# emsig/emg3d

Hardware: AMD Instinct MI355X
Metric: Mcells*smoother-iters/s (fp64) per multigrid cycle (higher is better)
Workload: dtype c128 (complex fp64)

## Files before the change

### emg3d_amd/csrc/kernels.hip

```cpp
#include <hip/hip_runtime.h>

#include <algorithm>
#include <climits>
#include <cstdio>
#include <cstdlib>
#include <cstring>
#include <string>
#include <type_traits>

#include "../../include/emg3d_amd.h"
#include "launch.h"

using emg::cplx;

namespace {

thread_local std::string g_err;

int fail(int code, const char *what)
{
    g_err = what;
    return code;
}

// ... 952 lines not shown
        else if (rq == 2) A.E(1)[A.idx(1, mk + 1, i1, i2)] = xq;
        else if (rq == 3) A.E(2)[A.idx(2, mk + 1, i1, i2 - 1)] = xq;
        else if (rq == 4) A.E(2)[A.idx(2, mk + 1, i1, i2)] = xq;
        else A.E(0)[A.idx(0, mk + 1, i1, i2)] = xq;
    }
    WSTAMP(5);
    __syncthreads();
    WSTAMP(6);
    {
        const int nst = (half ? nbb : nbt) - 1;
        if (chain_wave && nst > 0) {
            const int kb0 = half ? mk + 2 : mk - 1, dk = half ? 1 : -1;
            T *const rw = GH + (size_t)cl * rows * LW_ROW;
            const T v0 = rw[kb0 * LW_ROW + (lane & 3)];
            wide_chain<T, true>(rw, nbase, nrow, (unsigned)cl * 16, kb0 + dk, kb0, dk, nst, lane & 15, v0);
        }
    }
    WSTAMP(7);
    __syncthreads();
    WSTAMP(8);
    if (has && !isq) {
        const T *const hr = GH + ((size_t)ll * rows + k) * LW_ROW;
        T h[4], c[5], x[5];
#pragma unroll
        for (int q = 0; q < 4; ++q) h[q] = hr[q];
#pragma unroll
        for (int q = 0; q < 5; ++q) c[q] = r[q];
        emg::wide_x<T, 15>(Tk, c, h, x);
        emg::wide_block_scatter<T, DIR>(A, k, mir, i1, i2, x);
    }
    WSTAMP(9);
}

template <class T, int DIR>
__device__ __forceinline__ void stream_produce(const emg::Axes<T, DIR> &A, int colour, int cntp, int cntq, int n0p,
                                               int line0, int nl, int lpw, T *buf, int R, int chunk, int pt, int np,
                                               double *lfo = nullptr)
{
    const int n0 = A.n0();
    const int items = 2 * R * lpw;
    for (int it = pt; it < items; it += np) {
        int ll, row, half;
        if (DIR == 0) { row = it % R; ll = (it / R) % lpw; half = it / (R * lpw); }
        else { ll = it % lpw; row = (it / lpw) % R; half = it / (R * lpw); }
        const int i = chunk * R + row;
        const int k = half ? n0p - 1 - i : i;
        const int k0 = k, kt = half ? k - 1 : k;
        const int lid = line0 + min(ll, nl - 1);
        int i1, i2, l2;
        emg::line_of_thread<DIR>(colour, cntp, cntq, lid % cntp, lid / cntp, i1, i2, l2);
        T rhs[5];
        emg::line_rhs_t<T, DIR>(A, min(max(kt, 0), n0 - 1), i1, i2, rhs);
        rhs[0] = emg::line_rhs_e0<T, DIR>(A, min(max(k0, 0), n0 - 1), i1, i2);
        const double keep0 = (k0 >= 0 && k0 < n0) ? 1.0 : 0.0;
        const double keept = (kt >= 0 && kt < n0) ? 1.0 : 0.0;
        T *o = buf + ((size_t)(half * R + row) * lpw + ll) * 5;
        o[0] = keep0 * rhs[0];
#pragma unroll
        for (int r = 1; r < 5; ++r) o[r] = keept * rhs[r];
        if (lfo) {
            double c[8];
            emg::line_coupling<T, DIR>(A, k, i1, i2, half != 0, c);
            double *lo = lfo + ((size_t)(half * R + row) * lpw + ll) * 8;
#pragma unroll
            for (int r = 0; r < 8; ++r) lo[r] = c[r];
        }
    }
}

constexpr int stream_producers(int B, bool compact) { return (B >= 2 || compact) ? 384 : 256; }
constexpr int stream_depth(int dir, int B, bool compact) { return B >= 2 ? 2 : (compact && dir == 0) ? 8 : emg::LINE_PAD; }
constexpr bool stream_lf_ring(int B) { return B == 1; }

template <class T, int HALF, int RD, int B, class FT = T, class WT = T>
__device__ __forceinline__ void quad_forward_stream(int n0, int n0p, int nlines, int qline, int qend, int line0, int j,
                                                      const FT *fac, const double *lfac, WT *vec, size_t vstride,
                                                      size_t dummy_off, const T *ringbase, int lpw, int R, int nchunks,
                                                      const double *lfring)
{
    const HalfWalk<HALF> W(n0, n0p);
    const bool active = qline < qend;
    const int line = min(qline, qend - 1);
    const int ll = line - line0;
    const VecRef<WT> V = VecRef<WT>::global(vec, nlines);
    WT *const dummy = vec + dummy_off;
    WT *const dslot = dummy + ((threadIdx.x & 63) >> 2) * 5;
    constexpr bool LFR = stream_lf_ring(B);
    QuadRow<T, FT> ring[RD];
    using LAddr = LaneAddr<T, HALF, FT, WT>;
    const LAddr LA(fac, lfac, nlines, line, j, V);
    auto fetch = [&](QuadRow<T, FT> &q, int i) { q.template load<LAddr, false, !LFR>(LA, W.fwd(W.clampi(i))); };
#pragma unroll
    for (int d = 0; d < RD; ++d) fetch(ring[d], d);
    __syncthreads();
    T wsel[B], w4p[B];
#pragma unroll
    for (int b = 0; b < B; ++b) wsel[b] = w4p[b] = emg::zero<T>();
    const double nz = j != 0 ? 1.0 : 0.0, is0 = 1.0 - nz;
    const size_t srcelems = (size_t)2 * R * lpw * 5;
    const size_t bufelems = (size_t)B * srcelems;
    for (int c = 0; c < nchunks; ++c) {
        const T *const items = ringbase + (size_t)(c & 1) * bufelems + ((size_t)(HALF * R) * lpw + ll) * 5;
        const int iend = min((c + 1) * R, W.steps);
        for (int i0 = c * R; i0 < iend; i0 += RD) {
#pragma unroll
            for (int d = 0; d < RD; ++d) {
                const int k = W.fwd(i0 + d);
                QuadRow<T, FT> &q = ring[d];
                const T *const it = items + (size_t)(i0 + d - c * R) * lpw * 5;
                if constexpr (LFR)
                    q.take_b(lfring + (size_t)(c & 1) * ((size_t)2 * R * lpw * 8) +
                             ((size_t)(HALF * R + (i0 + d - c * R)) * lpw + ll) * 8, j);
                WT *const o4 = active ? LA.pv4(k) : dslot + 4;
                WT *const oj = active ? LA.pvj(k) : dslot + j;
#pragma unroll
                for (int b = 0; b < B; ++b) {
                    const T v = it[b * srcelems + j], v4 = it[b * srcelems + 4];
                    T wn, w4;
                    quad_forward_step(q, v, v4, nz, is0, wsel[b], w4p[b], wn, w4);
                    oj[b * vstride] = emg::narrow<WT>(wn);
                    o4[b * vstride] = emg::narrow<WT>(w4);
                }
                fetch(ring[d], i0 + d + RD);
            }
        }
        lds_barrier();
    }
}

template <class T, int DIR, class WT = T>
__device__ __forceinline__ void stream_produce_w(const WT *vec, int nlines, int n0, int n0p, int line0, int nl, int lpw,
                                                 T *buf, int R, int chunk, int pt, int np,
                                                 const emg::Axes<T, DIR> *A = nullptr, int colour = 0, int cntp = 0,
                                                 int cntq = 0, double *lfo = nullptr)
{
    const int mk = emg::line_mid(n0);
    const int items = 2 * R * lpw;
    for (int it = pt; it < items; it += np) {
        const int ll = it % lpw, row = (it / lpw) % R, half = it / (R * lpw);
        const int steps = half ? n0p - 2 - mk : mk;
        const int ic = max(min(chunk * R + row, steps - 1), 0);
        const int k = min(max(half ? mk + 2 + ic : mk - 1 - ic, half), n0p - 1);
        const int lid = line0 + min(ll, nl - 1);
        const WT *const r0 = vec + ((size_t)k * nlines + lid) * 5;
        const WT *const rt = vec + ((size_t)(half ? k - 1 : k) * nlines + lid) * 5;
        const WT a0 = r0[0], a1 = rt[1], a2 = rt[2], a3 = rt[3], a4 = rt[4];
        T *o = buf + ((size_t)(half * R + row) * lpw + ll) * 5;
        o[0] = emg::widen(a0); o[1] = emg::widen(a1); o[2] = emg::widen(a2); o[3] = emg::widen(a3); o[4] = emg::widen(a4);
        if (lfo) {
            int i1, i2, l2;
            emg::line_of_thread<DIR>(colour, cntp, cntq, lid % cntp, lid / cntp, i1, i2, l2);
            double c[8];
            emg::line_coupling<T, DIR>(*A, k, i1, i2, half != 0, c);
            double *lo = lfo + ((size_t)(half * R + row) * lpw + ll) * 8;
#pragma unroll
            for (int r = 0; r < 8; ++r) lo[r] = c[r];
        }
    }
}

template <class T, int DIR, int HALF, int RD, int B, class FT = T, class WT = T>
__device__ __forceinline__ void quad_backward_stream(const emg::Level<T> &L, int colour, int cntp, int cntq, int n0p, int qline,
                                                int qend, int line0, int j, const FT *fac, const double *lfac, WT *vec,
                                                size_t vstride, T *fdummy, size_t boff0, const T *ringbase, int lpw, int R,
                                                int nchunks, const double *lfring)
{
    const emg::Axes<T, DIR> A(L, boff0);
    const int n0 = A.n0();
    const HalfWalk<HALF> W(n0, n0p);
    const int mk = W.mk;
    const int nlines = cntp * cntq;
    const bool active = qline < qend;
    const int line = min(qline, qend - 1);
    const int ll = line - line0;
    const size_t bs = L.bstride;
    int i1, i2, lid;
    emg::line_of_thread<DIR>(colour, cntp, cntq, line % cntp, line / cntp, i1, i2, lid);
    const int cj = j == 0 ? 0 : (j <= 2 ? 1 : 2), dk = (j == 0 || HALF) ? 0 : 1, dk4 = HALF ? 0 : 1;
    const int d1 = j == 1 ? 1 : 0, d2 = j == 3 ? 1 : 0;
    T *const ej = A.E(cj) + A.idx(cj, dk, i1 - d1, i2 - d2);
    const long sj = (long)A.idx(cj, dk + 1, i1 - d1, i2 - d2) - (long)A.idx(cj, dk, i1 - d1, i2 - d2);
    T *const e4 = A.E(2) + A.idx(2, dk4, i1, i2);
    const long s4 = (long)A.idx(2, dk4 + 1, i1, i2) - (long)A.idx(2, dk4, i1, i2);
    T *const dslot = fdummy + ((threadIdx.x & 63) >> 2) * 5;
    T *const dj = dslot + j, *const d4 = dslot + 4;
    const size_t fstep = active ? bs : 0;

    const VecRef<WT> V = VecRef<WT>::global(vec, nlines);
    constexpr bool LFR = stream_lf_ring(B);
    QuadRow<T, FT> ring[RD];
// ... 48 lines not shown
                QuadRow<T, FT> &q = ring[d];
                const T *const it = items + (size_t)(i0 + d - c * R) * lpw * 5;
                if constexpr (LFR)
                    q.take_b(lfring + (size_t)(c & 1) * ((size_t)2 * R * lpw * 8) +
                             ((size_t)(HALF * R + (i0 + d - c * R)) * lpw + ll) * 8, j);
                const bool real_block = HALF ? k <= n0 - 1 : true;
                T *const oj = real_block ? pej : dj;
                T *const o4 = real_block ? pe4 : d4;
                const size_t ostep = real_block ? fstep : 0;
#pragma unroll
                for (int b = 0; b < B; ++b) {
                    const T wj = it[b * srcelems + j], w4 = it[b * srcelems + 4];
                    T xn, xn4;
                    quad_backward_step(q, wj, w4, nz, upA, upD, up04, up44, x0[b], x4[b], xmine[b], xn, xn4);
                    if (PAIRED && (d & 1) == 0) {
                        hold_j[b] = xn; hold_4[b] = xn4;
                    } else if (PAIRED) {
                        hold_oj[b * hold_step] = hold_j[b];
                        oj[b * ostep] = xn;
                        hold_o4[b * hold_step] = hold_4[b];
                        o4[b * ostep] = xn4;
                    } else {
                        oj[b * ostep] = xn;
                        o4[b * ostep] = xn4;
                    }
                }
                if (PAIRED && (d & 1) == 0) { hold_oj = oj; hold_o4 = o4; hold_step = ostep; }
                upA = q.bA; upD = q.bD; up04 = q.b04; up44 = q.d4;
                pej += incj;
                pe4 += inc4;
                fetch(ring[d], i0 + d + RD);
            }
        }
        lds_barrier();
    }
}

template <class T, int DIR, int B, bool COMPACT>
__global__ __launch_bounds__(128 + stream_producers(B, COMPACT), 1) void k_line_stream(emg::Level<T> L, int colour, int cntp, int cntq, int n0p,
                                                                    int lpw, int R, const void *facv, const double *lfac,
                                                                    T *vecT, size_t vstrideT, size_t boff0)
{
    constexpr int RD = stream_depth(DIR, B, COMPACT), NPROD = stream_producers(B, COMPACT);
    constexpr bool LFR = stream_lf_ring(B);
    using FT = typename std::conditional<COMPACT, typename emg::compact_of<T>::type, T>::type;
    using WT = FT;
    const FT *const fac = reinterpret_cast<const FT *>(facv);
    WT *const vec = reinterpret_cast<WT *>(vecT);
    const size_t vstride = vstrideT * (sizeof(T) / sizeof(WT));
    const size_t dummy_off = vstrideT - emg::LINE_DUMMY;
    T *const fdummy = vecT + dummy_off;
    extern __shared__ double2 ls_smem[];
    const int nlines = cntp * cntq;
    const int line0 = blockIdx.x * lpw;
    const int nl = min(lpw, nlines - line0);
    T *const ringbase = reinterpret_cast<T *>(ls_smem);
    const size_t srcelems = (size_t)2 * R * lpw * 5, bufelems = (size_t)B * srcelems;
    double *const lfring = LFR ? reinterpret_cast<double *>(ringbase + 2 * bufelems) : nullptr;
    const size_t lfelems = (size_t)2 * R * lpw * 8;
    const int n0 = DIR == 0 ? L.nx : DIR == 1 ? L.ny : L.nz;
    const int mk = emg::line_mid(n0);
    const int smax = max(mk, n0p - 2 - mk);
    const int nchunks = (smax + R - 1) / R;
    const int wave = threadIdx.x >> 6;
    if (wave >= 2) {
        const int pt = threadIdx.x - 128;
#pragma unroll 1
        for (int b = 0; b < B; ++b) {
            const emg::Axes<T, DIR> A(L, boff0 + b * L.bstride);
            const VecRef<WT> V = VecRef<WT>::global(vec + b * vstride, nlines);
            for (int ll = pt; ll < nl; ll += NPROD) {
                const int lid = line0 + ll;
                int i1, i2, l2;
                emg::line_of_thread<DIR>(colour, cntp, cntq, lid % cntp, lid / cntp, i1, i2, l2);
                T rhs[5];
                emg::line_rhs<T, DIR>(A, mk, i1, i2, rhs);
#pragma unroll
                for (int r = 0; r < 4; ++r) *V.p(mk, lid, r) = emg::narrow<WT>(rhs[r]);
                *V.p4(mk, lid) = emg::narrow<WT>(rhs[4]);
                *V.p(mk + 1, lid, 0) = emg::narrow<WT>(emg::line_rhs_e0<T, DIR>(A, min(mk + 1, n0 - 1), i1, i2));
            }
            stream_produce<T, DIR>(A, colour, cntp, cntq, n0p, line0, nl, lpw, ringbase + b * srcelems, R, 0, pt, NPROD,
                                   (LFR && b == 0) ? lfring : nullptr);
        }
        __syncthreads();
        for (int c = 0; c < nchunks; ++c) {
            if (c + 1 < nchunks) {
#pragma unroll 1
                for (int b = 0; b < B; ++b) {
                    const emg::Axes<T, DIR> A(L, boff0 + b * L.bstride);
                    stream_produce<T, DIR>(A, colour, cntp, cntq, n0p, line0, nl, lpw,
                                           ringbase + (size_t)((c + 1) & 1) * bufelems + b * srcelems, R, c + 1, pt, NPROD,
                                           (LFR && b == 0) ? lfring + (size_t)((c + 1) & 1) * lfelems : nullptr);
                }
            }
            lds_barrier();
        }
        __syncthreads();
        const emg::Axes<T, DIR> A0(L, boff0);
#pragma unroll 1
        for (int b = 0; b < B; ++b)
            stream_produce_w<T, DIR, WT>(vec + b * vstride, nlines, n0, n0p, line0, nl, lpw, ringbase + b * srcelems, R, 0, pt, NPROD,
                                         &A0, colour, cntp, cntq, (LFR && b == 0) ? lfring : nullptr);
        __syncthreads();
        for (int c = 0; c < nchunks; ++c) {
            if (c + 1 < nchunks) {
#pragma unroll 1
                for (int b = 0; b < B; ++b)
                    stream_produce_w<T, DIR, WT>(vec + b * vstride, nlines, n0, n0p, line0, nl, lpw,
                                                 ringbase + (size_t)((c + 1) & 1) * bufelems + b * srcelems, R, c + 1, pt, NPROD,
                                                 &A0, colour, cntp, cntq,
                                                 (LFR && b == 0) ? lfring + (size_t)((c + 1) & 1) * lfelems : nullptr);
            }
            lds_barrier();
        }
        return;
    }
    const int half = wave & 1;
    const int qline = line0 + ((threadIdx.x & 63) >> 2), j = threadIdx.x & 3;
    const int qend = line0 + nl;
    if (half == 0) quad_forward_stream<T, 0, RD, B, FT, WT>(n0, n0p, nlines, qline, qend, line0, j, fac, lfac, vec, vstride, dummy_off, ringbase, lpw, R, nchunks, lfring);
    else quad_forward_stream<T, 1, RD, B, FT, WT>(n0, n0p, nlines, qline, qend, line0, j, fac, lfac, vec, vstride, dummy_off, ringbase, lpw, R, nchunks, lfring);
    __syncthreads();
    if (half == 0) quad_backward_stream<T, DIR, 0, RD, B, FT, WT>(L, colour, cntp, cntq, n0p, qline, qend, line0, j, fac, lfac, vec, vstride, fdummy, boff0, ringbase, lpw, R, nchunks, lfring);
    else quad_backward_stream<T, DIR, 1, RD, B, FT, WT>(L, colour, cntp, cntq, n0p, qline, qend, line0, j, fac, lfac, vec, vstride, fdummy, boff0, ringbase, lpw, R, nchunks, lfring);
}

#pragma clang fp contract(fast)

template <class T, bool ROLL>
__global__ __launch_bounds__(256) void k_residual(emg::Level<T> L0, T *rx, T *ry, T *rz, double *partial, int nzb, int zb)
{
    const int b = blockIdx.z / nzb;
    const emg::Level<T> L = emg::source_level(L0, b);
    if (rx) { rx += b * L0.bstride; ry += b * L0.bstride; rz += b * L0.bstride; }
    const int ix = blockIdx.x * blockDim.x + threadIdx.x;
    const int iy = blockIdx.y * blockDim.y + threadIdx.y;
    const int z0 = (blockIdx.z - b * nzb) * zb, z1 = min(z0 + zb, L.nz + 1);
    double acc = 0.0;
    if (ix <= L.nx && iy <= L.ny) {
        if constexpr (ROLL) acc = emg::residual_column<T>(L, rx, ry, rz, ix, iy, z0, z1);
        else for (int iz = z0; iz < z1; ++iz) acc += emg::residual_cell<T>(L, rx, ry, rz, ix, iy, iz);
    }
    if (partial) {
        for (int off = 32; off > 0; off >>= 1) acc += __shfl_down(acc, off, 64);
        __shared__ double wsum[4];
        const int tid = threadIdx.y * blockDim.x + threadIdx.x;
// ... 567 lines not shown
    {"line_wide_bt", &g_line_wide_bt},
    {"line_compact", &g_line_compact, -1, 1},
    {"point_compact", &g_point_compact, -1, 1},
};
constexpr int N_OPTIONS = sizeof(g_options) / sizeof(g_options[0]);
static int g_options_generation = 0;

int emg3d_option_count(void) { return N_OPTIONS; }
const char *emg3d_option_name(int i) { return (i >= 0 && i < N_OPTIONS) ? g_options[i].name : nullptr; }

int emg3d_set_option(const char *name, int value)
{
    if (!name) return fail(EMG3D_ERR_BADARG, "set_option: null name");
    for (const OptionEntry &o : g_options) {
        if (std::strcmp(name, o.name)) continue;
        if (o.value == &g_residual_zb && value < 1) value = 1;
        bool ok = value >= o.lo && value <= o.hi;
        if (o.value == &g_line_lpw) ok = value == 0 || value == 4 || value == 8 || value == 16 || value == 32;
        if (o.value == &g_line_stream_r) ok = ok && value % emg::LINE_PAD == 0;
        if (o.value == &g_line_wide_bt) ok = value == 0 || value == 192 || value == 256;
        if (!ok) {
            g_err = std::string("set_option: ") + name + " = " + std::to_string(value) + " is not an admissible value";
            return EMG3D_ERR_BADARG;
        }
        if (*o.value != value) ++g_options_generation;
        *o.value = value;
        return 0;
    }
    return fail(EMG3D_ERR_BADARG, "set_option: unknown option");
}

int emg3d_options_generation(void) { return g_options_generation; }

#ifdef EMG_WIDE_STAMPS
int emg3d_debug_wide_stamps(unsigned long long *out)
{
    return (int)hipMemcpyFromSymbol(out, HIP_SYMBOL(g_wide_stamps), sizeof(unsigned long long) * 32);
}
#endif

const char *emg3d_line_kernel_name(int lr, int nx, int ny, int nz, int is_complex, int batch)
{
    if (lr < 1 || lr > 3 || nx < 2 || ny < 2 || nz < 2) return "";
    const emg::LineClass lc = emg::line_class(lr - 1, nx, ny, nz, 3);
    if (lc.lines <= 0) return "";
    if (line_wide_used(lr - 1, nx, ny, nz)) return "k_line_wide";
    const LinePlan P = is_complex ? line_plan<cplx>(lc, batch > 1 ? batch : 1) : line_plan<double>(lc, batch > 1 ? batch : 1);
    switch (P.kind) {
    case LK_STREAM: return "k_line_stream";
    case LK_COLOUR: return "k_line_colour";
    default: return "k_line_rhs+k_line_forward+k_line_backward";
    }
}

int emg3d_get_option(const char *name)
{
    if (name)
        for (const OptionEntry &o : g_options)
            if (!std::strcmp(name, o.name)) return *o.value;
    return -1;
}

int emg3d_device_count(void)
{
    int n = 0;
    if (hipGetDeviceCount(&n) != hipSuccess) return 0;
// ... 384 lines not shown
```

### emg3d_amd/csrc/stencil.h

```cpp
#pragma once
#include "cplx.h"

namespace emg {

template <class T> struct Level {
    int nx, ny, nz;
    T *ex, *ey, *ez;
    const T *sx, *sy, *sz;
    const T *eta_x, *eta_y, *eta_z;
    const double *zeta;
    const double *ihx, *ihy, *ihz;
    int batch = 1;
    size_t bstride = 0;
    int flags = 0;
};
constexpr int LEVEL_ETA_IMAG = 1;
constexpr int LEVEL_LINE_COMPACT = 2;
constexpr int LEVEL_POINT_COMPACT = 4;
template <class T> EMG_HD Level<T> source_level(Level<T> L, int b)
{
    size_t o = (size_t)b * L.bstride;
#if defined(__HIP_DEVICE_COMPILE__)
    o = ((size_t)__builtin_amdgcn_readfirstlane((unsigned)(o >> 32)) << 32) | (size_t)__builtin_amdgcn_readfirstlane((unsigned)o);
#endif
// ... 635 lines not shown
    const double mxyLzm = k10 * (z100 + z000), mxyRzm = k11 * (z110 + z010);
    const double myxLzp = k00 * (z011 + z001), myxRzp = k01 * (z111 + z101);
    const double mxyLzp = k10 * (z101 + z001), mxyRzp = k11 * (z111 + z011);

    const T st0 = A.eta(0, i0m, i1, i2) + A.eta(0, i0m, i1, i2m) + A.eta(0, i0m, i1m, i2) +
                  A.eta(0, i0m, i1m, i2m);
    const T st2 = A.eta(1, i0, i1m, i2) + A.eta(1, i0, i1m, i2m) + A.eta(1, i0m, i1m, i2) +
                  A.eta(1, i0m, i1m, i2m);
    const T st3 = A.eta(1, i0, i1, i2) + A.eta(1, i0, i1, i2m) + A.eta(1, i0m, i1, i2) +
                  A.eta(1, i0m, i1, i2m);
    const T st4 = A.eta(2, i0, i1, i2m) + A.eta(2, i0, i1m, i2m) + A.eta(2, i0m, i1, i2m) +
                  A.eta(2, i0m, i1m, i2m);
    const T st5 = A.eta(2, i0, i1, i2) + A.eta(2, i0, i1m, i2) + A.eta(2, i0m, i1, i2) +
                  A.eta(2, i0m, i1m, i2);

    dg[0] = (mzyRxm * h11 + mzyLxm * h10 + myzRxm * h21 + myzLxm * h20) - 0.25 * st0;
    dg[1] = (mzxRym * h01 + mzxLym * h00 + mxzRym * h21 + mxzLym * h20) - 0.25 * st2;
    dg[2] = (mzxRyp * h01 + mzxLyp * h00 + mxzRyp * h21 + mxzLyp * h20) - 0.25 * st3;
    dg[3] = (myxRzm * h01 + myxLzm * h00 + mxyRzm * h11 + mxyLzm * h10) - 0.25 * st4;
    dg[4] = (myxRzp * h01 + myxLzp * h00 + mxyRzp * h11 + mxyLzp * h10) - 0.25 * st5;

    mid[1][0] = -mzyLxm * h00; mid[2][0] = mzyRxm * h00; mid[3][0] = -myzLxm * h00; mid[4][0] = myzRxm * h00;
    mid[2][1] = 0.0;
    mid[3][1] = -mxzLym * h10; mid[4][1] = mxzRym * h10;
    mid[3][2] = mxzLyp * h11; mid[4][2] = -mxzRyp * h11;
    mid[4][3] = 0.0;

    left0[0] = 0.0;
    left0[1] = mzyLxm * h00; left0[2] = -mzyRxm * h00; left0[3] = myzLxm * h00; left0[4] = -myzRxm * h00;
    leftd[0] = 0.0;
    leftd[1] = -mzxLym * h00; leftd[2] = -mzxLyp * h00; leftd[3] = -myxLzm * h00; leftd[4] = -myxLzp * h00;
}

template <class T, int DIR>
EMG_HD T line_rhs_e0(const Axes<T, DIR> &A, int k, int i1, int i2)
{
    const int i0m = k;
    const int i1m = i1 - 1, i1p = i1 + 1, i2m = i2 - 1, i2p = i2 + 1;
    const double h10 = A.ih1()[i1m], h11 = A.ih1()[i1];
    const double h20 = A.ih2()[i2m], h21 = A.ih2()[i2];
    const double k10 = 0.5 * h10, k11 = 0.5 * h11, k20 = 0.5 * h20, k21 = 0.5 * h21;
    const double z000 = A.zeta(i0m, i1m, i2m), z010 = A.zeta(i0m, i1, i2m);
    const double z001 = A.zeta(i0m, i1m, i2), z011 = A.zeta(i0m, i1, i2);
    const double mzyLxm = k10 * (z001 + z000), mzyRxm = k11 * (z011 + z010);
    const double myzLxm = k20 * (z010 + z000), myzRxm = k21 * (z011 + z001);
    T r0 = A.s(0, i0m, i1, i2);
    r0 += (mzyRxm * h11) * A.e(0, i0m, i1p, i2);
    r0 += (mzyLxm * h10) * A.e(0, i0m, i1m, i2);
    r0 += (myzRxm * h21) * A.e(0, i0m, i1, i2p);
    r0 += (myzLxm * h20) * A.e(0, i0m, i1, i2m);
    return r0;
}
template <class T, int DIR>
EMG_HD void line_rhs_t(const Axes<T, DIR> &A, int k, int i1, int i2, T (&rhs)[5])
{
    const int n0 = A.n0();
    const int i0m = k;
    const int i0 = (k + 1 < n0 - 1) ? k + 1 : n0 - 1;
    const int i1m = i1 - 1, i1p = i1 + 1, i2m = i2 - 1, i2p = i2 + 1;
    const double h00 = A.ih0()[i0m], h01 = A.ih0()[i0];
    const double h10 = A.ih1()[i1m], h11 = A.ih1()[i1];
    const double h20 = A.ih2()[i2m], h21 = A.ih2()[i2];
    const double k00 = 0.5 * h00, k01 = 0.5 * h01, k10 = 0.5 * h10, k11 = 0.5 * h11;
    const double k20 = 0.5 * h20, k21 = 0.5 * h21;

    const double z000 = A.zeta(i0m, i1m, i2m), z010 = A.zeta(i0m, i1, i2m);
    const double z001 = A.zeta(i0m, i1m, i2), z011 = A.zeta(i0m, i1, i2);
    const double z100 = A.zeta(i0, i1m, i2m), z110 = A.zeta(i0, i1, i2m);
    const double z101 = A.zeta(i0, i1m, i2), z111 = A.zeta(i0, i1, i2);
    const double mzxLym = k00 * (z001 + z000), mzxRym = k01 * (z101 + z100);
    const double mxzLym = k20 * (z100 + z000), mxzRym = k21 * (z101 + z001);
    const double mzxLyp = k00 * (z011 + z010), mzxRyp = k01 * (z111 + z110);
    const double mxzLyp = k20 * (z110 + z010), mxzRyp = k21 * (z111 + z011);
    const double myxLzm = k00 * (z010 + z000), myxRzm = k01 * (z110 + z100);
    const double mxyLzm = k10 * (z100 + z000), mxyRzm = k11 * (z110 + z010);
    const double myxLzp = k00 * (z011 + z001), myxRzp = k01 * (z111 + z101);
    const double mxyLzp = k10 * (z101 + z001), mxyRzp = k11 * (z111 + z011);

    rhs[1] = A.s(1, i0, i1m, i2);
    rhs[2] = A.s(1, i0, i1, i2);
    rhs[3] = A.s(2, i0, i1, i2m);
    rhs[4] = A.s(2, i0, i1, i2);

    rhs[1] += h10 * (mzxRym * A.e(0, i0, i1m, i2) - mzxLym * A.e(0, i0m, i1m, i2) +
                     mxzRym * A.e(2, i0, i1m, i2) - mxzLym * A.e(2, i0, i1m, i2m));
    rhs[1] += (mxzRym * h21) * A.e(1, i0, i1m, i2p);
    rhs[1] += (mxzLym * h20) * A.e(1, i0, i1m, i2m);

    rhs[2] += h11 * (mzxLyp * A.e(0, i0m, i1p, i2) - mzxRyp * A.e(0, i0, i1p, i2) +
                     mxzLyp * A.e(2, i0, i1p, i2m) - mxzRyp * A.e(2, i0, i1p, i2));
    rhs[2] += (mxzRyp * h21) * A.e(1, i0, i1, i2p);
    rhs[2] += (mxzLyp * h20) * A.e(1, i0, i1, i2m);

    rhs[3] += h20 * (myxRzm * A.e(0, i0, i1, i2m) - myxLzm * A.e(0, i0m, i1, i2m) +
                     mxyRzm * A.e(1, i0, i1, i2m) - mxyLzm * A.e(1, i0, i1m, i2m));
    rhs[3] += (mxyRzm * h11) * A.e(2, i0, i1p, i2m);
    rhs[3] += (mxyLzm * h10) * A.e(2, i0, i1m, i2m);

    rhs[4] += h21 * (myxLzp * A.e(0, i0m, i1, i2p) - myxRzp * A.e(0, i0, i1, i2p) +
                     mxyLzp * A.e(1, i0, i1m, i2p) - mxyRzp * A.e(1, i0, i1, i2p));
    rhs[4] += (mxyRzp * h11) * A.e(2, i0, i1p, i2);
    rhs[4] += (mxyLzp * h10) * A.e(2, i0, i1m, i2);
    if (k == n0 - 1) rhs[1] = rhs[2] = rhs[3] = rhs[4] = zero<T>();
}
template <class T, int DIR>
EMG_HD void line_rhs(const Axes<T, DIR> &A, int k, int i1, int i2, T (&rhs)[5])
{
    line_rhs_t<T, DIR>(A, k, i1, i2, rhs);
    rhs[0] = line_rhs_e0<T, DIR>(A, k, i1, i2);
}


template <class T, int DIR>
EMG_HD void line_coupling(const Axes<T, DIR> &A, int k, int i1, int i2, bool mirrored, double (&c)[8])
{
    const int n0 = A.n0();
    const int kk = k < 0 ? 0 : (k > n0 - 1 ? n0 - 1 : k);
    const int i1m = i1 - 1, i2m = i2 - 1;
    const double h00 = A.ih0()[kk];
    const double h10 = A.ih1()[i1m], h11 = A.ih1()[i1];
    const double h20 = A.ih2()[i2m], h21 = A.ih2()[i2];
    const double k00 = 0.5 * h00, k10 = 0.5 * h10, k11 = 0.5 * h11, k20 = 0.5 * h20, k21 = 0.5 * h21;
    const double z000 = A.zeta(kk, i1m, i2m), z010 = A.zeta(kk, i1, i2m);
    const double z001 = A.zeta(kk, i1m, i2), z011 = A.zeta(kk, i1, i2);
    const double mzyLxm = k10 * (z001 + z000), mzyRxm = k11 * (z011 + z010);
    const double myzLxm = k20 * (z010 + z000), myzRxm = k21 * (z011 + z001);
    const double mzxLym = k00 * (z001 + z000), mzxLyp = k00 * (z011 + z010);
    const double myxLzm = k00 * (z010 + z000), myxLzp = k00 * (z011 + z001);
    const bool any = mirrored ? (k >= 1 && k < n0 - 1) : (k >= 1 && k <= n0 - 1);
    const double a0 = mzyLxm * h00, a1 = mzyRxm * h00, a2 = myzLxm * h00, a3 = myzRxm * h00;
    c[0] = any ? (mirrored ? -a0 : a0) : 0.0;
    c[1] = any ? (mirrored ? a1 : -a1) : 0.0;
    c[2] = any ? (mirrored ? -a2 : a2) : 0.0;
    c[3] = any ? (mirrored ? a3 : -a3) : 0.0;
    c[4] = any ? -(mzxLym * h00) : 0.0;
    c[5] = any ? -(mzxLyp * h00) : 0.0;
    c[6] = any ? -(myxLzm * h00) : 0.0;
    c[7] = any ? -(myxLzp * h00) : 0.0;
}

template <class T> EMG_HD void ldlt5(const T (&S)[5][5], int nrows, T (&C)[10], T (&dinv)[5])
{
#pragma unroll
    for (int r = 0; r < 5; ++r) {
        if (r < nrows) {
            T u[5];
#pragma unroll
            for (int m = 0; m < r; ++m) {
                T t = S[r][m];
#pragma unroll
                for (int kk = 0; kk < m; ++kk) t -= u[kk] * C[tri(m, kk)];
                u[m] = t;
                C[tri(r, m)] = t * dinv[m];
            }
            T d = S[r][r];
#pragma unroll
            for (int kk = 0; kk < r; ++kk) d -= u[kk] * C[tri(r, kk)];
            dinv[r] = recip(d);
        } else {
            dinv[r] = T(1.0);
#pragma unroll
            for (int m = 0; m < r; ++m) C[tri(r, m)] = zero<T>();
        }
    }
}

template <class T> EMG_HD void ldlt5_solve(const T (&C)[10], const T (&dinv)[5], T (&v)[5])
{
#pragma unroll
    for (int r = 1; r < 5; ++r) {
#pragma unroll
// ... 815 lines not shown
```

Measured before the change: 3850.

## Software-pipeline stream producer loads one item ahead for single-batch path

Splits the line RHS, e0 and coupling computations into separate load and compute phases held in register structs. In the B==1 streaming producer, the global loads for the next item (or the next chunk's first item) are issued before the current item's values are computed and stored, so global memory latency overlaps with arithmetic and the LDS barrier wait. This raises register pressure because the staging structs hold roughly 30 complex values, which may reduce occupancy. Optional timestamp instrumentation is added behind a compile flag.

```diff
diff --git a/emg3d_amd/csrc/kernels.hip b/emg3d_amd/csrc/kernels.hip
--- a/emg3d_amd/csrc/kernels.hip
+++ b/emg3d_amd/csrc/kernels.hip
@@ -1008,39 +1008,81 @@
     WSTAMP(9);
 }
 
+#ifdef EMG_STREAM_STAMPS
+__device__ unsigned long long g_stream_stamps[2 * 2 * 64 * 2];
+#define SSTAMP(who, pass, c, w)                                                                         \
+    do {                                                                                                \
+        if (blockIdx.x == 0 && threadIdx.x == ((who) ? 128 : 0) && (c) < 64)                            \
+            g_stream_stamps[((((who) * 2 + (pass)) * 64) + (c)) * 2 + (w)] = __builtin_amdgcn_s_memtime(); \
+    } while (0)
+#else
+#define SSTAMP(who, pass, c, w)
+#endif
+
+template <class T> struct StreamRhsIn {
+    emg::LineRhsTIn<T> t;
+    emg::LineRhsE0In<T> e0;
+    emg::LineCouplingIn<T> cp;
+};
+template <int DIR> __device__ __forceinline__ void stream_item(int it, int R, int lpw, int &ll, int &row, int &half)
+{
+    if (DIR == 0) { row = it % R; ll = (it / R) % lpw; half = it / (R * lpw); }
+    else { ll = it % lpw; row = (it / lpw) % R; half = it / (R * lpw); }
+}
+template <class T, int DIR>
+__device__ __forceinline__ void stream_rhs_load(const emg::Axes<T, DIR> &A, int colour, int cntp, int cntq, int n0p,
+                                                int line0, int nl, int lpw, int R, int chunk, int it, bool lf,
+                                                StreamRhsIn<T> &in)
+{
+    const int n0 = A.n0();
+    int ll, row, half;
+    stream_item<DIR>(it, R, lpw, ll, row, half);
+    const int i = chunk * R + row;
+    const int k = half ? n0p - 1 - i : i;
+    const int k0 = k, kt = half ? k - 1 : k;
+    const int lid = line0 + min(ll, nl - 1);
+    int i1, i2, l2;
+    emg::line_of_thread<DIR>(colour, cntp, cntq, lid % cntp, lid / cntp, i1, i2, l2);
+    emg::line_rhs_t_load<T, DIR>(A, min(max(kt, 0), n0 - 1), i1, i2, in.t);
+    emg::line_rhs_e0_load<T, DIR>(A, min(max(k0, 0), n0 - 1), i1, i2, in.e0);
+    if (lf) emg::line_coupling_load<T, DIR>(A, k, i1, i2, half != 0, in.cp);
+}
+template <class T, int DIR>
+__device__ __forceinline__ void stream_rhs_store(int n0, int n0p, int lpw, T *buf, int R, int chunk, int it,
+                                                 const StreamRhsIn<T> &in, double *lfo)
+{
+    int ll, row, half;
+    stream_item<DIR>(it, R, lpw, ll, row, half);
+    const int i = chunk * R + row;
+    const int k = half ? n0p - 1 - i : i;
+    const int k0 = k, kt = half ? k - 1 : k;
+    T rhs[5];
+    emg::line_rhs_t_compute<T>(in.t, rhs);
+    rhs[0] = emg::line_rhs_e0_compute<T>(in.e0);
+    const double keep0 = (k0 >= 0 && k0 < n0) ? 1.0 : 0.0;
+    const double keept = (kt >= 0 && kt < n0) ? 1.0 : 0.0;
+    T *o = buf + ((size_t)(half * R + row) * lpw + ll) * 5;
+    o[0] = keep0 * rhs[0];
+#pragma unroll
+    for (int r = 1; r < 5; ++r) o[r] = keept * rhs[r];
+    if (lfo) {
+        double c[8];
+        emg::line_coupling_compute<T>(in.cp, half != 0, c);
+        double *lo = lfo + ((size_t)(half * R + row) * lpw + ll) * 8;
+#pragma unroll
+        for (int r = 0; r < 8; ++r) lo[r] = c[r];
+    }
+}
 template <class T, int DIR>
 __device__ __forceinline__ void stream_produce(const emg::Axes<T, DIR> &A, int colour, int cntp, int cntq, int n0p,
                                                int line0, int nl, int lpw, T *buf, int R, int chunk, int pt, int np,
                                                double *lfo = nullptr)
 {
-    const int n0 = A.n0();
     const int items = 2 * R * lpw;
     for (int it = pt; it < items; it += np) {
-        int ll, row, half;
-        if (DIR == 0) { row = it % R; ll = (it / R) % lpw; half = it / (R * lpw); }
-        else { ll = it % lpw; row = (it / lpw) % R; half = it / (R * lpw); }
-        const int i = chunk * R + row;
-        const int k = half ? n0p - 1 - i : i;
-        const int k0 = k, kt = half ? k - 1 : k;
-        const int lid = line0 + min(ll, nl - 1);
-        int i1, i2, l2;
-        emg::line_of_thread<DIR>(colour, cntp, cntq, lid % cntp, lid / cntp, i1, i2, l2);
-        T rhs[5];
-        emg::line_rhs_t<T, DIR>(A, min(max(kt, 0), n0 - 1), i1, i2, rhs);
-        rhs[0] = emg::line_rhs_e0<T, DIR>(A, min(max(k0, 0), n0 - 1), i1, i2);
-        const double keep0 = (k0 >= 0 && k0 < n0) ? 1.0 : 0.0;
-        const double keept = (kt >= 0 && kt < n0) ? 1.0 : 0.0;
-        T *o = buf + ((size_t)(half * R + row) * lpw + ll) * 5;
-        o[0] = keep0 * rhs[0];
-#pragma unroll
-        for (int r = 1; r < 5; ++r) o[r] = keept * rhs[r];
-        if (lfo) {
-            double c[8];
-            emg::line_coupling<T, DIR>(A, k, i1, i2, half != 0, c);
-            double *lo = lfo + ((size_t)(half * R + row) * lpw + ll) * 8;
-#pragma unroll
-            for (int r = 0; r < 8; ++r) lo[r] = c[r];
-        }
+        StreamRhsIn<T> in;
+        stream_rhs_load<T, DIR>(A, colour, cntp, cntq, n0p, line0, nl, lpw, R, chunk, it, lfo != nullptr, in);
+        stream_rhs_store<T, DIR>(A.n0(), n0p, lpw, buf, R, chunk, it, in, lfo);
     }
 }
 
@@ -1100,38 +1142,61 @@
                 fetch(ring[d], i0 + d + RD);
             }
         }
+        SSTAMP(0, 0, c, 0);
         lds_barrier();
-    }
-}
-
+        SSTAMP(0, 0, c, 1);
+    }
+}
+
+template <class T, class WT> struct StreamWIn {
+    WT a0, a1, a2, a3, a4;
+    emg::LineCouplingIn<T> cp;
+};
+template <class T, int DIR, class WT>
+__device__ __forceinline__ void stream_w_load(const WT *vec, int nlines, int n0, int n0p, int line0, int nl, int lpw, int R,
+                                              int chunk, int it, const emg::Axes<T, DIR> *A, int colour, int cntp, int cntq,
+                                              bool lf, StreamWIn<T, WT> &in)
+{
+    const int mk = emg::line_mid(n0);
+    const int ll = it % lpw, row = (it / lpw) % R, half = it / (R * lpw);
+    const int steps = half ? n0p - 2 - mk : mk;
+    const int ic = max(min(chunk * R + row, steps - 1), 0);
+    const int k = min(max(half ? mk + 2 + ic : mk - 1 - ic, half), n0p - 1);
+    const int lid = line0 + min(ll, nl - 1);
+    const WT *const r0 = vec + ((size_t)k * nlines + lid) * 5;
+    const WT *const rt = vec + ((size_t)(half ? k - 1 : k) * nlines + lid) * 5;
+    in.a0 = r0[0]; in.a1 = rt[1]; in.a2 = rt[2]; in.a3 = rt[3]; in.a4 = rt[4];
+    if (lf) {
+        int i1, i2, l2;
+        emg::line_of_thread<DIR>(colour, cntp, cntq, lid % cntp, lid / cntp, i1, i2, l2);
+        emg::line_coupling_load<T, DIR>(*A, k, i1, i2, half != 0, in.cp);
+    }
+}
+template <class T, class WT>
+__device__ __forceinline__ void stream_w_store(int lpw, T *buf, int R, int it, const StreamWIn<T, WT> &in, double *lfo)
+{
+    const int ll = it % lpw, row = (it / lpw) % R, half = it / (R * lpw);
+    T *o = buf + ((size_t)(half * R + row) * lpw + ll) * 5;
+    o[0] = emg::widen(in.a0); o[1] = emg::widen(in.a1); o[2] = emg::widen(in.a2); o[3] = emg::widen(in.a3); o[4] = emg::widen(in.a4);
+    if (lfo) {
+        double c[8];
+        emg::line_coupling_compute<T>(in.cp, half != 0, c);
+        double *lo = lfo + ((size_t)(half * R + row) * lpw + ll) * 8;
+#pragma unroll
+        for (int r = 0; r < 8; ++r) lo[r] = c[r];
+    }
+}
 template <class T, int DIR, class WT = T>
 __device__ __forceinline__ void stream_produce_w(const WT *vec, int nlines, int n0, int n0p, int line0, int nl, int lpw,
                                                  T *buf, int R, int chunk, int pt, int np,
                                                  const emg::Axes<T, DIR> *A = nullptr, int colour = 0, int cntp = 0,
                                                  int cntq = 0, double *lfo = nullptr)
 {
-    const int mk = emg::line_mid(n0);
     const int items = 2 * R * lpw;
     for (int it = pt; it < items; it += np) {
-        const int ll = it % lpw, row = (it / lpw) % R, half = it / (R * lpw);
-        const int steps = half ? n0p - 2 - mk : mk;
-        const int ic = max(min(chunk * R + row, steps - 1), 0);
-        const int k = min(max(half ? mk + 2 + ic : mk - 1 - ic, half), n0p - 1);
-        const int lid = line0 + min(ll, nl - 1);
-        const WT *const r0 = vec + ((size_t)k * nlines + lid) * 5;
-        const WT *const rt = vec + ((size_t)(half ? k - 1 : k) * nlines + lid) * 5;
-        const WT a0 = r0[0], a1 = rt[1], a2 = rt[2], a3 = rt[3], a4 = rt[4];
-        T *o = buf + ((size_t)(half * R + row) * lpw + ll) * 5;
-        o[0] = emg::widen(a0); o[1] = emg::widen(a1); o[2] = emg::widen(a2); o[3] = emg::widen(a3); o[4] = emg::widen(a4);
-        if (lfo) {
-            int i1, i2, l2;
-            emg::line_of_thread<DIR>(colour, cntp, cntq, lid % cntp, lid / cntp, i1, i2, l2);
-            double c[8];
-            emg::line_coupling<T, DIR>(*A, k, i1, i2, half != 0, c);
-            double *lo = lfo + ((size_t)(half * R + row) * lpw + ll) * 8;
-#pragma unroll
-            for (int r = 0; r < 8; ++r) lo[r] = c[r];
-        }
+        StreamWIn<T, WT> in;
+        stream_w_load<T, DIR, WT>(vec, nlines, n0, n0p, line0, nl, lpw, R, chunk, it, A, colour, cntp, cntq, lfo != nullptr, in);
+        stream_w_store<T, WT>(lpw, buf, R, it, in, lfo);
     }
 }
 
@@ -1246,7 +1311,9 @@
                 fetch(ring[d], i0 + d + RD);
             }
         }
+        SSTAMP(0, 1, c, 0);
         lds_barrier();
+        SSTAMP(0, 1, c, 1);
     }
 }
 
@@ -1297,9 +1364,27 @@
             stream_produce<T, DIR>(A, colour, cntp, cntq, n0p, line0, nl, lpw, ringbase + b * srcelems, R, 0, pt, NPROD,
                                    (LFR && b == 0) ? lfring : nullptr);
         }
+        const int items = 2 * R * lpw;
+        const emg::Axes<T, DIR> A0(L, boff0);
+        StreamRhsIn<T> rin;
+        if constexpr (B == 1)
+            if (nchunks > 1 && pt < items)
+                stream_rhs_load<T, DIR>(A0, colour, cntp, cntq, n0p, line0, nl, lpw, R, 1, pt, LFR, rin);
         __syncthreads();
         for (int c = 0; c < nchunks; ++c) {
-            if (c + 1 < nchunks) {
+            if constexpr (B == 1) {
+                if (c + 1 < nchunks) {
+#pragma unroll 1
+                    for (int it = pt; it < items; it += NPROD) {
+                        stream_rhs_store<T, DIR>(n0, n0p, lpw, ringbase + (size_t)((c + 1) & 1) * bufelems, R, c + 1, it, rin,
+                                                 LFR ? lfring + (size_t)((c + 1) & 1) * lfelems : nullptr);
+                        const bool more = it + NPROD < items;
+                        const int cn = more ? c + 1 : c + 2, itn = more ? it + NPROD : pt;
+                        if (cn < nchunks)
+                            stream_rhs_load<T, DIR>(A0, colour, cntp, cntq, n0p, line0, nl, lpw, R, cn, itn, LFR, rin);
+                    }
+                }
+            } else if (c + 1 < nchunks) {
 #pragma unroll 1
                 for (int b = 0; b < B; ++b) {
                     const emg::Axes<T, DIR> A(L, boff0 + b * L.bstride);
@@ -1308,17 +1393,35 @@
                                            (LFR && b == 0) ? lfring + (size_t)((c + 1) & 1) * lfelems : nullptr);
                 }
             }
+            SSTAMP(1, 0, c, 0);
             lds_barrier();
+            SSTAMP(1, 0, c, 1);
         }
         __syncthreads();
-        const emg::Axes<T, DIR> A0(L, boff0);
 #pragma unroll 1
         for (int b = 0; b < B; ++b)
             stream_produce_w<T, DIR, WT>(vec + b * vstride, nlines, n0, n0p, line0, nl, lpw, ringbase + b * srcelems, R, 0, pt, NPROD,
                                          &A0, colour, cntp, cntq, (LFR && b == 0) ? lfring : nullptr);
+        StreamWIn<T, WT> win;
+        if constexpr (B == 1)
+            if (nchunks > 1 && pt < items)
+                stream_w_load<T, DIR, WT>(vec, nlines, n0, n0p, line0, nl, lpw, R, 1, pt, &A0, colour, cntp, cntq, LFR, win);
         __syncthreads();
         for (int c = 0; c < nchunks; ++c) {
-            if (c + 1 < nchunks) {
+            if constexpr (B == 1) {
+                if (c + 1 < nchunks) {
+#pragma unroll 1
+                    for (int it = pt; it < items; it += NPROD) {
+                        stream_w_store<T, WT>(lpw, ringbase + (size_t)((c + 1) & 1) * bufelems, R, it, win,
+                                              LFR ? lfring + (size_t)((c + 1) & 1) * lfelems : nullptr);
+                        const bool more = it + NPROD < items;
+                        const int cn = more ? c + 1 : c + 2, itn = more ? it + NPROD : pt;
+                        if (cn < nchunks)
+                            stream_w_load<T, DIR, WT>(vec, nlines, n0, n0p, line0, nl, lpw, R, cn, itn, &A0, colour, cntp, cntq,
+                                                      LFR, win);
+                    }
+                }
+            } else if (c + 1 < nchunks) {
 #pragma unroll 1
                 for (int b = 0; b < B; ++b)
                     stream_produce_w<T, DIR, WT>(vec + b * vstride, nlines, n0, n0p, line0, nl, lpw,
@@ -1326,7 +1429,9 @@
                                                  &A0, colour, cntp, cntq,
                                                  (LFR && b == 0) ? lfring + (size_t)((c + 1) & 1) * lfelems : nullptr);
             }
+            SSTAMP(1, 1, c, 0);
             lds_barrier();
+            SSTAMP(1, 1, c, 1);
         }
         return;
     }
@@ -1960,6 +2065,13 @@
 
 int emg3d_options_generation(void) { return g_options_generation; }
 
+#ifdef EMG_STREAM_STAMPS
+int emg3d_debug_stream_stamps(unsigned long long *out)
+{
+    return (int)hipMemcpyFromSymbol(out, HIP_SYMBOL(g_stream_stamps), sizeof(unsigned long long) * 2 * 2 * 64 * 2);
+}
+#endif
+
 #ifdef EMG_WIDE_STAMPS
 int emg3d_debug_wide_stamps(unsigned long long *out)
 {
diff --git a/emg3d_amd/csrc/stencil.h b/emg3d_amd/csrc/stencil.h
--- a/emg3d_amd/csrc/stencil.h
+++ b/emg3d_amd/csrc/stencil.h
@@ -691,42 +691,101 @@
     leftd[1] = -mzxLym * h00; leftd[2] = -mzxLyp * h00; leftd[3] = -myxLzm * h00; leftd[4] = -myxLzp * h00;
 }
 
+template <class T> struct LineRhsE0In {
+    double h10, h11, h20, h21;
+    double z000, z010, z001, z011;
+    T s0;
+    T e_1p, e_1m, e_2p, e_2m;
+};
+template <class T, int DIR>
+EMG_HD void line_rhs_e0_load(const Axes<T, DIR> &A, int k, int i1, int i2, LineRhsE0In<T> &in)
+{
+    const int i0m = k;
+    const int i1m = i1 - 1, i1p = i1 + 1, i2m = i2 - 1, i2p = i2 + 1;
+    in.h10 = A.ih1()[i1m]; in.h11 = A.ih1()[i1];
+    in.h20 = A.ih2()[i2m]; in.h21 = A.ih2()[i2];
+    in.z000 = A.zeta(i0m, i1m, i2m); in.z010 = A.zeta(i0m, i1, i2m);
+    in.z001 = A.zeta(i0m, i1m, i2); in.z011 = A.zeta(i0m, i1, i2);
+    in.s0 = A.s(0, i0m, i1, i2);
+    in.e_1p = A.e(0, i0m, i1p, i2);
+    in.e_1m = A.e(0, i0m, i1m, i2);
+    in.e_2p = A.e(0, i0m, i1, i2p);
+    in.e_2m = A.e(0, i0m, i1, i2m);
+}
+template <class T> EMG_HD T line_rhs_e0_compute(const LineRhsE0In<T> &in)
+{
+    const double h10 = in.h10, h11 = in.h11;
+    const double h20 = in.h20, h21 = in.h21;
+    const double k10 = 0.5 * h10, k11 = 0.5 * h11, k20 = 0.5 * h20, k21 = 0.5 * h21;
+    const double z000 = in.z000, z010 = in.z010;
+    const double z001 = in.z001, z011 = in.z011;
+    const double mzyLxm = k10 * (z001 + z000), mzyRxm = k11 * (z011 + z010);
+    const double myzLxm = k20 * (z010 + z000), myzRxm = k21 * (z011 + z001);
+    T r0 = in.s0;
+    r0 += (mzyRxm * h11) * in.e_1p;
+    r0 += (mzyLxm * h10) * in.e_1m;
+    r0 += (myzRxm * h21) * in.e_2p;
+    r0 += (myzLxm * h20) * in.e_2m;
+    return r0;
+}
 template <class T, int DIR>
 EMG_HD T line_rhs_e0(const Axes<T, DIR> &A, int k, int i1, int i2)
 {
-    const int i0m = k;
-    const int i1m = i1 - 1, i1p = i1 + 1, i2m = i2 - 1, i2p = i2 + 1;
-    const double h10 = A.ih1()[i1m], h11 = A.ih1()[i1];
-    const double h20 = A.ih2()[i2m], h21 = A.ih2()[i2];
-    const double k10 = 0.5 * h10, k11 = 0.5 * h11, k20 = 0.5 * h20, k21 = 0.5 * h21;
-    const double z000 = A.zeta(i0m, i1m, i2m), z010 = A.zeta(i0m, i1, i2m);
-    const double z001 = A.zeta(i0m, i1m, i2), z011 = A.zeta(i0m, i1, i2);
-    const double mzyLxm = k10 * (z001 + z000), mzyRxm = k11 * (z011 + z010);
-    const double myzLxm = k20 * (z010 + z000), myzRxm = k21 * (z011 + z001);
-    T r0 = A.s(0, i0m, i1, i2);
-    r0 += (mzyRxm * h11) * A.e(0, i0m, i1p, i2);
-    r0 += (mzyLxm * h10) * A.e(0, i0m, i1m, i2);
-    r0 += (myzRxm * h21) * A.e(0, i0m, i1, i2p);
-    r0 += (myzLxm * h20) * A.e(0, i0m, i1, i2m);
-    return r0;
-}
+    LineRhsE0In<T> in;
+    line_rhs_e0_load<T, DIR>(A, k, i1, i2, in);
+    return line_rhs_e0_compute<T>(in);
+}
+
+template <class T> struct LineRhsTIn {
+    double h00, h01, h10, h11, h20, h21;
+    double z000, z010, z001, z011, z100, z110, z101, z111;
+    T s1m, s1, s2m, s2;
+    T e0_1m, e0m_1m, e0_1p, e0m_1p;
+    T e0_2m, e0m_2m, e0_2p, e0m_2p;
+    T e1_1m_2p, e1_1m_2m, e1_2p, e1_2m;
+    T e2_1m, e2_1m_2m, e2_1p_2m, e2_1p;
+    bool last;
+};
 template <class T, int DIR>
-EMG_HD void line_rhs_t(const Axes<T, DIR> &A, int k, int i1, int i2, T (&rhs)[5])
+EMG_HD void line_rhs_t_load(const Axes<T, DIR> &A, int k, int i1, int i2, LineRhsTIn<T> &in)
 {
     const int n0 = A.n0();
     const int i0m = k;
     const int i0 = (k + 1 < n0 - 1) ? k + 1 : n0 - 1;
     const int i1m = i1 - 1, i1p = i1 + 1, i2m = i2 - 1, i2p = i2 + 1;
-    const double h00 = A.ih0()[i0m], h01 = A.ih0()[i0];
-    const double h10 = A.ih1()[i1m], h11 = A.ih1()[i1];
-    const double h20 = A.ih2()[i2m], h21 = A.ih2()[i2];
+    in.h00 = A.ih0()[i0m]; in.h01 = A.ih0()[i0];
+    in.h10 = A.ih1()[i1m]; in.h11 = A.ih1()[i1];
+    in.h20 = A.ih2()[i2m]; in.h21 = A.ih2()[i2];
+    in.z000 = A.zeta(i0m, i1m, i2m); in.z010 = A.zeta(i0m, i1, i2m);
+    in.z001 = A.zeta(i0m, i1m, i2); in.z011 = A.zeta(i0m, i1, i2);
+    in.z100 = A.zeta(i0, i1m, i2m); in.z110 = A.zeta(i0, i1, i2m);
+    in.z101 = A.zeta(i0, i1m, i2); in.z111 = A.zeta(i0, i1, i2);
+    in.s1m = A.s(1, i0, i1m, i2);
+    in.s1 = A.s(1, i0, i1, i2);
+    in.s2m = A.s(2, i0, i1, i2m);
+    in.s2 = A.s(2, i0, i1, i2);
+    in.e0_1m = A.e(0, i0, i1m, i2); in.e0m_1m = A.e(0, i0m, i1m, i2);
+    in.e0_1p = A.e(0, i0, i1p, i2); in.e0m_1p = A.e(0, i0m, i1p, i2);
+    in.e0_2m = A.e(0, i0, i1, i2m); in.e0m_2m = A.e(0, i0m, i1, i2m);
+    in.e0_2p = A.e(0, i0, i1, i2p); in.e0m_2p = A.e(0, i0m, i1, i2p);
+    in.e1_1m_2p = A.e(1, i0, i1m, i2p); in.e1_1m_2m = A.e(1, i0, i1m, i2m);
+    in.e1_2p = A.e(1, i0, i1, i2p); in.e1_2m = A.e(1, i0, i1, i2m);
+    in.e2_1m = A.e(2, i0, i1m, i2); in.e2_1m_2m = A.e(2, i0, i1m, i2m);
+    in.e2_1p_2m = A.e(2, i0, i1p, i2m); in.e2_1p = A.e(2, i0, i1p, i2);
+    in.last = k == n0 - 1;
+}
+template <class T> EMG_HD void line_rhs_t_compute(const LineRhsTIn<T> &in, T (&rhs)[5])
+{
+    const double h00 = in.h00, h01 = in.h01;
+    const double h10 = in.h10, h11 = in.h11;
+    const double h20 = in.h20, h21 = in.h21;
     const double k00 = 0.5 * h00, k01 = 0.5 * h01, k10 = 0.5 * h10, k11 = 0.5 * h11;
     const double k20 = 0.5 * h20, k21 = 0.5 * h21;
 
-    const double z000 = A.zeta(i0m, i1m, i2m), z010 = A.zeta(i0m, i1, i2m);
-    const double z001 = A.zeta(i0m, i1m, i2), z011 = A.zeta(i0m, i1, i2);
-    const double z100 = A.zeta(i0, i1m, i2m), z110 = A.zeta(i0, i1, i2m);
-    const double z101 = A.zeta(i0, i1m, i2), z111 = A.zeta(i0, i1, i2);
+    const double z000 = in.z000, z010 = in.z010;
+    const double z001 = in.z001, z011 = in.z011;
+    const double z100 = in.z100, z110 = in.z110;
+    const double z101 = in.z101, z111 = in.z111;
     const double mzxLym = k00 * (z001 + z000), mzxRym = k01 * (z101 + z100);
     const double mxzLym = k20 * (z100 + z000), mxzRym = k21 * (z101 + z001);
     const double mzxLyp = k00 * (z011 + z010), mzxRyp = k01 * (z111 + z110);
@@ -736,31 +795,38 @@
     const double myxLzp = k00 * (z011 + z001), myxRzp = k01 * (z111 + z101);
     const double mxyLzp = k10 * (z101 + z001), mxyRzp = k11 * (z111 + z011);
 
-    rhs[1] = A.s(1, i0, i1m, i2);
-    rhs[2] = A.s(1, i0, i1, i2);
-    rhs[3] = A.s(2, i0, i1, i2m);
-    rhs[4] = A.s(2, i0, i1, i2);
-
-    rhs[1] += h10 * (mzxRym * A.e(0, i0, i1m, i2) - mzxLym * A.e(0, i0m, i1m, i2) +
-                     mxzRym * A.e(2, i0, i1m, i2) - mxzLym * A.e(2, i0, i1m, i2m));
-    rhs[1] += (mxzRym * h21) * A.e(1, i0, i1m, i2p);
-    rhs[1] += (mxzLym * h20) * A.e(1, i0, i1m, i2m);
-
-    rhs[2] += h11 * (mzxLyp * A.e(0, i0m, i1p, i2) - mzxRyp * A.e(0, i0, i1p, i2) +
-                     mxzLyp * A.e(2, i0, i1p, i2m) - mxzRyp * A.e(2, i0, i1p, i2));
-    rhs[2] += (mxzRyp * h21) * A.e(1, i0, i1, i2p);
-    rhs[2] += (mxzLyp * h20) * A.e(1, i0, i1, i2m);
-
-    rhs[3] += h20 * (myxRzm * A.e(0, i0, i1, i2m) - myxLzm * A.e(0, i0m, i1, i2m) +
-                     mxyRzm * A.e(1, i0, i1, i2m) - mxyLzm * A.e(1, i0, i1m, i2m));
-    rhs[3] += (mxyRzm * h11) * A.e(2, i0, i1p, i2m);
-    rhs[3] += (mxyLzm * h10) * A.e(2, i0, i1m, i2m);
-
-    rhs[4] += h21 * (myxLzp * A.e(0, i0m, i1, i2p) - myxRzp * A.e(0, i0, i1, i2p) +
-                     mxyLzp * A.e(1, i0, i1m, i2p) - mxyRzp * A.e(1, i0, i1, i2p));
-    rhs[4] += (mxyRzp * h11) * A.e(2, i0, i1p, i2);
-    rhs[4] += (mxyLzp * h10) * A.e(2, i0, i1m, i2);
-    if (k == n0 - 1) rhs[1] = rhs[2] = rhs[3] = rhs[4] = zero<T>();
+    rhs[1] = in.s1m;
+    rhs[2] = in.s1;
+    rhs[3] = in.s2m;
+    rhs[4] = in.s2;
+
+    rhs[1] += h10 * (mzxRym * in.e0_1m - mzxLym * in.e0m_1m +
+                     mxzRym * in.e2_1m - mxzLym * in.e2_1m_2m);
+    rhs[1] += (mxzRym * h21) * in.e1_1m_2p;
+    rhs[1] += (mxzLym * h20) * in.e1_1m_2m;
+
+    rhs[2] += h11 * (mzxLyp * in.e0m_1p - mzxRyp * in.e0_1p +
+                     mxzLyp * in.e2_1p_2m - mxzRyp * in.e2_1p);
+    rhs[2] += (mxzRyp * h21) * in.e1_2p;
+    rhs[2] += (mxzLyp * h20) * in.e1_2m;
+
+    rhs[3] += h20 * (myxRzm * in.e0_2m - myxLzm * in.e0m_2m +
+                     mxyRzm * in.e1_2m - mxyLzm * in.e1_1m_2m);
+    rhs[3] += (mxyRzm * h11) * in.e2_1p_2m;
+    rhs[3] += (mxyLzm * h10) * in.e2_1m_2m;
+
+    rhs[4] += h21 * (myxLzp * in.e0m_2p - myxRzp * in.e0_2p +
+                     mxyLzp * in.e1_1m_2p - mxyRzp * in.e1_2p);
+    rhs[4] += (mxyRzp * h11) * in.e2_1p;
+    rhs[4] += (mxyLzp * h10) * in.e2_1m;
+    if (in.last) rhs[1] = rhs[2] = rhs[3] = rhs[4] = zero<T>();
+}
+template <class T, int DIR>
+EMG_HD void line_rhs_t(const Axes<T, DIR> &A, int k, int i1, int i2, T (&rhs)[5])
+{
+    LineRhsTIn<T> in;
+    line_rhs_t_load<T, DIR>(A, k, i1, i2, in);
+    line_rhs_t_compute<T>(in, rhs);
 }
 template <class T, int DIR>
 EMG_HD void line_rhs(const Axes<T, DIR> &A, int k, int i1, int i2, T (&rhs)[5])
@@ -770,23 +836,37 @@
 }
 
 
+template <class T> struct LineCouplingIn {
+    double h00, h10, h11, h20, h21;
+    double z000, z010, z001, z011;
+    bool any;
+};
 template <class T, int DIR>
-EMG_HD void line_coupling(const Axes<T, DIR> &A, int k, int i1, int i2, bool mirrored, double (&c)[8])
+EMG_HD void line_coupling_load(const Axes<T, DIR> &A, int k, int i1, int i2, bool mirrored, LineCouplingIn<T> &in)
 {
     const int n0 = A.n0();
     const int kk = k < 0 ? 0 : (k > n0 - 1 ? n0 - 1 : k);
     const int i1m = i1 - 1, i2m = i2 - 1;
-    const double h00 = A.ih0()[kk];
-    const double h10 = A.ih1()[i1m], h11 = A.ih1()[i1];
-    const double h20 = A.ih2()[i2m], h21 = A.ih2()[i2];
+    in.h00 = A.ih0()[kk];
+    in.h10 = A.ih1()[i1m]; in.h11 = A.ih1()[i1];
+    in.h20 = A.ih2()[i2m]; in.h21 = A.ih2()[i2];
+    in.z000 = A.zeta(kk, i1m, i2m); in.z010 = A.zeta(kk, i1, i2m);
+    in.z001 = A.zeta(kk, i1m, i2); in.z011 = A.zeta(kk, i1, i2);
+    in.any = mirrored ? (k >= 1 && k < n0 - 1) : (k >= 1 && k <= n0 - 1);
+}
+template <class T> EMG_HD void line_coupling_compute(const LineCouplingIn<T> &in, bool mirrored, double (&c)[8])
+{
+    const double h00 = in.h00;
+    const double h10 = in.h10, h11 = in.h11;
+    const double h20 = in.h20, h21 = in.h21;
     const double k00 = 0.5 * h00, k10 = 0.5 * h10, k11 = 0.5 * h11, k20 = 0.5 * h20, k21 = 0.5 * h21;
-    const double z000 = A.zeta(kk, i1m, i2m), z010 = A.zeta(kk, i1, i2m);
-    const double z001 = A.zeta(kk, i1m, i2), z011 = A.zeta(kk, i1, i2);
+    const double z000 = in.z000, z010 = in.z010;
+    const double z001 = in.z001, z011 = in.z011;
     const double mzyLxm = k10 * (z001 + z000), mzyRxm = k11 * (z011 + z010);
     const double myzLxm = k20 * (z010 + z000), myzRxm = k21 * (z011 + z001);
     const double mzxLym = k00 * (z001 + z000), mzxLyp = k00 * (z011 + z010);
     const double myxLzm = k00 * (z010 + z000), myxLzp = k00 * (z011 + z001);
-    const bool any = mirrored ? (k >= 1 && k < n0 - 1) : (k >= 1 && k <= n0 - 1);
+    const bool any = in.any;
     const double a0 = mzyLxm * h00, a1 = mzyRxm * h00, a2 = myzLxm * h00, a3 = myzRxm * h00;
     c[0] = any ? (mirrored ? -a0 : a0) : 0.0;
     c[1] = any ? (mirrored ? a1 : -a1) : 0.0;
@@ -796,6 +876,13 @@
     c[5] = any ? -(mzxLyp * h00) : 0.0;
     c[6] = any ? -(myxLzm * h00) : 0.0;
     c[7] = any ? -(myxLzp * h00) : 0.0;
+}
+template <class T, int DIR>
+EMG_HD void line_coupling(const Axes<T, DIR> &A, int k, int i1, int i2, bool mirrored, double (&c)[8])
+{
+    LineCouplingIn<T> in;
+    line_coupling_load<T, DIR>(A, k, i1, i2, mirrored, in);
+    line_coupling_compute<T>(in, mirrored, c);
 }
 
 template <class T> EMG_HD void ldlt5(const T (&S)[5][5], int nrows, T (&C)[10], T (&dinv)[5])
```

New measurement: 3882, median of 6. No clear change (+0.8%).
